# williamyang1991/VToonify

Hardware: NVIDIA H100
Metric: frames/sec at 576x1024 (higher is better)
Workload: dtype bf16x3 (fp32 operands split into bf16 hi+lo, 3 tensor-core products, fp32 accumulate)

## Files before the change

vtoonify_b200/csrc/conv_tc.cu:

```cuda
#include "tc_common.cuh"
#include <cuda_bf16.h>
#include <mutex>

using namespace vt_tc;

int vt_validate_conv_desc(const vt_conv_desc* d, const char* who);
extern int g_upfirdn_tiled;
extern int g_smalln_is;
extern int g_fir4;
extern int g_instnorm_chunks;
extern int g_rs_kernel;
int vt_conv_rs_takes(const vt_conv_desc* d);
int vt_conv_rs_run(const vt_conv_desc* d, void* stream);

namespace {

constexpr int TILE_W = 8, TILE_H = 16, TILE_M = 128;
constexpr int KCH = 32;
constexpr int MAX_SMEM = 227 * 1024;
constexpr int MAX_BLOCK_N = 128;
constexpr int MAX_ACC_COLS = 128;
constexpr int STATS_WARPS = 8;

struct TcArgs {
  CUtensorMap in_map[2][4];
  CUtensorMap w_map;
  int n_src, kchunks[2], coff[2];
  int n_steps;
  int8_t step_view[VT_MAX_TAPS], step_vx[VT_MAX_TAPS], step_vy[VT_MAX_TAPS];
  int16_t step_w[VT_MAX_TAPS];
  int step_aoff[VT_MAX_TAPS];
  int n_phase;
  int tgroup;
  int halo, halo_x0, halo_y0, halo_w;
  int n_hv, hv_view[4], hv_x0[4], hv_y0[4], hv_off[4], hv_bytes[4], a_rows;
  uint16_t step_sbo[VT_MAX_TAPS];
  int a_stages, b_stages, a_stage_bytes, b_stage_bytes, a_tx_bytes, b_tx_bytes;
  int block_n, n_tiles, tiles_x, tiles_y, B, total_tiles;
  int Ho, Wo, Cout, wB, out_cpitch;
  const float* bias;
  const float* noise;
  const float* noise_w;
  const float* res;
  float* out;
  int64_t out_sb, out_sy, out_sx, phase_off[4];
  int64_t pix_sb, pix_sy, pix_sx, phase_pix[4];
  int act, round_tf32;
  float slope, gain, alpha, beta;
  const float* rgb_w; const float* rgb_bias; const float* rgb_skip; const float* rgb_skip_kernel; float* rgb_out;
  const float* slope_vec;
  const float* src_scale[2];
  const float* src_affine[2];
  int src_cn[2];
  int64_t sc_sb, sc_sy, sc_sx;
  int in_w, in_h;
  int mma_n;
  int m_major;
  float* stats_ws;
  float acc_scale;
};

constexpr int TC_THREADS = 384;
constexpr int XFORM_WARPS = 3;
constexpr int CONSUMERS = 2;
constexpr int RELEASE_ARRIVALS = CONSUMERS * 4;

enum TcOp : int {
  OP_TF32 = 0,
  OP_BF16 = 1,
  OP_F16 = 2,
  OP_BF16_NSTACK = 3,
};

template <int NW, bool F16>
__device__ __forceinline__ void wgmma_split(float* acc, uint64_t a, uint64_t b, uint32_t accumulate) {
  if constexpr (NW == 32) {
    if constexpr (F16) wgmma_f16_n32(acc, a, b, accumulate); else wgmma_bf16_n32(acc, a, b, accumulate);
  } else if constexpr (NW == 64) {
    if constexpr (F16) wgmma_f16_n64(acc, a, b, accumulate); else wgmma_bf16_n64(acc, a, b, accumulate);
  } else {
    if constexpr (F16) wgmma_f16_n128(acc, a, b, accumulate); else wgmma_bf16_n128(acc, a, b, accumulate);
  }
}

template <int NW, int OP>
__device__ __forceinline__ void mma_step(float* acc, uint64_t adesc, uint64_t bdesc, uint32_t first) {
  if constexpr (OP == OP_TF32) {
    if constexpr (NW == 32) {
      wgmma_tf32_n32(acc, adesc, bdesc, first ^ 1u); wgmma_tf32_n32(acc, adesc + 2, bdesc + 2, 1);
      wgmma_tf32_n32(acc, adesc + 4, bdesc + 4, 1); wgmma_tf32_n32(acc, adesc + 6, bdesc + 6, 1);
    } else if constexpr (NW == 64) {
      wgmma_tf32_n64(acc, adesc, bdesc, first ^ 1u); wgmma_tf32_n64(acc, adesc + 2, bdesc + 2, 1);
      wgmma_tf32_n64(acc, adesc + 4, bdesc + 4, 1); wgmma_tf32_n64(acc, adesc + 6, bdesc + 6, 1);
    } else {
      wgmma_tf32_n128(acc, adesc, bdesc, first ^ 1u); wgmma_tf32_n128(acc, adesc + 2, bdesc + 2, 1);
      wgmma_tf32_n128(acc, adesc + 4, bdesc + 4, 1); wgmma_tf32_n128(acc, adesc + 6, bdesc + 6, 1);
    }
  } else {
    constexpr bool nstack = OP == OP_BF16_NSTACK;
    constexpr int ao[6] = {0, 2, 4, 6, 0, 2};
    constexpr int bo[6] = {0, 2, 0, 2, 4, 6};
#pragma unroll
    for (int i = 0; i < (nstack ? 4 : 6); ++i)
      wgmma_split<NW, OP == OP_F16>(acc, adesc + (uint64_t)ao[i], bdesc + (uint64_t)(nstack ? ao[i] : bo[i]), i == 0 ? (first ^ 1u) : 1u);
  }
}

template <int NW, int MT, int OP>
__global__ void __launch_bounds__(TC_THREADS, 1)
conv_tc_kernel(const __grid_constant__ TcArgs p) {
  static_assert(MT * NW <= MAX_ACC_COLS && (MT == 1 || MT == 2 || MT == 4), "accumulators of one work item exceed the register plan");
  static_assert(OP != OP_BF16_NSTACK || NW == 64, "the N-stacked form is the Cout == 32 layer at MMA N = 64");
  constexpr bool SPLIT = OP != OP_TF32;
  extern __shared__ uint8_t smem_raw[];
  const uint32_t smem_base = (smem_u32(smem_raw) + 1023u) & ~1023u;
  const uint32_t a_base = smem_base;
  const uint32_t b_base = a_base + (uint32_t)p.a_stages * p.a_stage_bytes;
  const uint32_t bar_base = b_base + (uint32_t)p.b_stages * p.b_stage_bytes;
  auto a_full = [&](int i) { return bar_base + 8u * i; };
  auto a_empty = [&](int i) { return bar_base + 64u + 8u * i; };
  auto b_full = [&](int i) { return bar_base + 128u + 8u * i; };
  auto b_empty = [&](int i) { return bar_base + 192u + 8u * i; };
  auto a_ready = [&](int i) { return bar_base + 256u + 8u * i; };

  const int warp = threadIdx.x >> 5, lane = threadIdx.x & 31;
  const int wg = threadIdx.x >> 7;

  if (warp == 0 && lane == 0) {
    for (int s = 0; s < p.n_src; ++s)
      for (int v = 0; v < 4; ++v) tma_prefetch_desc(&p.in_map[s][v]);
    tma_prefetch_desc(&p.w_map);
  }
  if (warp == 1 && lane == 0) {
    for (int i = 0; i < p.a_stages; ++i) { mbar_init(a_full(i), 1); mbar_init(a_empty(i), RELEASE_ARRIVALS); mbar_init(a_ready(i), XFORM_WARPS); }
    for (int i = 0; i < p.b_stages; ++i) { mbar_init(b_full(i), 1); mbar_init(b_empty(i), RELEASE_ARRIVALS); }
    fence_barrier_init();
    fence_proxy_async_smem();
  }
  __syncthreads();

  const int m_tiles = p.B * p.tiles_y * p.tiles_x;
  const int tiles_per_img = p.tiles_y * p.tiles_x;
  constexpr int item_w = TILE_W * MT;

  if (wg == 0) {
    if (warp == 0) {
      int a_st = 0, b_st = 0;
      uint32_t a_par = 0, b_par = 0;
      for (int tile = blockIdx.x; tile < p.total_tiles; tile += gridDim.x) {
        const int n_tile = p.m_major ? tile % p.n_tiles : tile / m_tiles, m = p.m_major ? tile / p.n_tiles : tile % m_tiles;
        const int b = m / tiles_per_img, rem = m % tiles_per_img;
        const int oy0 = (rem / p.tiles_x) * TILE_H, ox0 = (rem % p.tiles_x) * item_w;
        const int n0 = n_tile * p.block_n;
        const int wb = p.wB > 1 ? b : 0;
        for (int s = 0; s < p.n_src; ++s) {
          for (int kc = 0; kc < p.kchunks[s]; ++kc) {
            const int c0 = kc * KCH;
            if (p.halo) {
              mbar_wait(a_empty(a_st), a_par ^ 1);
              if (elect_one()) {
                const uint32_t st = a_base + a_st * p.a_stage_bytes;
                mbar_arrive_expect_tx(a_full(a_st), (uint32_t)p.a_tx_bytes);
                for (int v = 0; v < p.n_hv; ++v)
                  tma_load_4d(st + p.hv_off[v], &p.in_map[s][p.hv_view[v]], a_full(a_st), c0, ox0 + p.hv_x0[v], oy0 + p.hv_y0[v], b);
              }
              __syncwarp();
              if (++a_st == p.a_stages) { a_st = 0; a_par ^= 1; }
            }
            int gj = 0;
            for (int j = 0; j < p.n_steps; ++j) {
              if (!p.halo) {
                mbar_wait(a_empty(a_st), a_par ^ 1);
                if (elect_one()) {
// ... 6 lines not shown
              }
              if (gj == 0) {
                mbar_wait(b_empty(b_st), b_par ^ 1);
                if (elect_one()) {
                  const int wc = SPLIT ? (p.coff[s] + c0) * 2 : p.coff[s] + c0;
                  mbar_arrive_expect_tx(b_full(b_st), (uint32_t)p.b_tx_bytes);
                  tma_load_4d(b_base + b_st * p.b_stage_bytes, &p.w_map, b_full(b_st), wc, OP == OP_BF16_NSTACK ? 0 : n0, p.step_w[j], wb);
                }
                __syncwarp();
                if (++b_st == p.b_stages) { b_st = 0; b_par ^= 1; }
              }
              if (++gj == p.tgroup) gj = 0;
            }
          }
        }
      }
    } else if constexpr (SPLIT) {
      const int t = (warp - 1) * 32 + lane;
      const int rows = p.a_rows;
      int a_st = 0;
      uint32_t a_par = 0;
      const int bw = p.halo ? p.halo_w : TILE_W;
      for (int tile = blockIdx.x; tile < p.total_tiles; tile += gridDim.x) {
        const int m = p.m_major ? tile / p.n_tiles : tile % m_tiles;
        const int b = m / tiles_per_img, rem = m % tiles_per_img;
        const int oy0 = (rem / p.tiles_x) * TILE_H, ox0 = (rem % p.tiles_x) * item_w;
        for (int s = 0; s < p.n_src; ++s) {
          const float* sc = p.src_scale[s];
          const float* aff = p.src_affine[s];
          for (int kc = 0; kc < p.kchunks[s]; ++kc) {
            const float4* affp = aff ? reinterpret_cast<const float4*>(aff + ((int64_t)b * p.src_cn[s] + kc * KCH) * 2) : nullptr;
            const int loads = p.halo ? 1 : p.n_steps;
            for (int l = 0; l < loads; ++l) {
              mbar_wait(a_full(a_st), a_par);
              const uint32_t stage = a_base + a_st * p.a_stage_bytes;
              const int bx0 = ox0 + (p.halo ? p.halo_x0 : p.step_vx[l]), by0 = oy0 + (p.halo ? p.halo_y0 : p.step_vy[l]);
              for (int r = t; r < rows; r += 32 * XFORM_WARPS) {
                const uint32_t row = stage + (uint32_t)r * 128u;
                const uint32_t ph = (row >> 7) & 7u;
                float f[32];
#pragma unroll
                for (int j = 0; j < 8; ++j) {
                  float4 v;
                  asm volatile("ld.shared.v4.f32 {%0, %1, %2, %3}, [%4];" : "=f"(v.x), "=f"(v.y), "=f"(v.z), "=f"(v.w) : "r"(row + ((j ^ ph) << 4)));
                  f[4 * j] = v.x; f[4 * j + 1] = v.y; f[4 * j + 2] = v.z; f[4 * j + 3] = v.w;
                }
                if (sc || aff) {
// ... 24 lines not shown
                    const __nv_bfloat162 h2 = __floats2bfloat162_rn(f[2 * i], f[2 * i + 1]);
                    hi[i] = *reinterpret_cast<const uint32_t*>(&h2);
                    const float r0 = f[2 * i] - __uint_as_float(hi[i] << 16), r1 = f[2 * i + 1] - __uint_as_float(hi[i] & 0xffff0000u);
                    const __nv_bfloat162 l2 = __floats2bfloat162_rn(r0, r1);
                    lo[i] = *reinterpret_cast<const uint32_t*>(&l2);
                  }
                }
#pragma unroll
                for (int m4 = 0; m4 < 4; ++m4) {
                  asm volatile("st.shared.v4.b32 [%0], {%1, %2, %3, %4};" ::"r"(row + ((m4 ^ ph) << 4)), "r"(hi[4 * m4]), "r"(hi[4 * m4 + 1]), "r"(hi[4 * m4 + 2]), "r"(hi[4 * m4 + 3]) : "memory");
                  asm volatile("st.shared.v4.b32 [%0], {%1, %2, %3, %4};" ::"r"(row + (((m4 + 4) ^ ph) << 4)), "r"(lo[4 * m4]), "r"(lo[4 * m4 + 1]), "r"(lo[4 * m4 + 2]), "r"(lo[4 * m4 + 3]) : "memory");
                }
              }
              fence_proxy_async_smem();
              __syncwarp();
              if (lane == 0) mbar_arrive(a_ready(a_st));
              if (++a_st == p.a_stages) { a_st = 0; a_par ^= 1; }
            }
          }
        }
      }
    }
  } else {
    const int c = wg - 1;
    const int tw_ = (threadIdx.x & 127) >> 5;
    const bool leader = lane == 0;
    const int qd = lane & 3;
    float acc[MT][NW / 2];
#pragma unroll
    for (int g = 0; g < MT; ++g)
#pragma unroll
      for (int i = 0; i < NW / 2; ++i) acc[g][i] = 0.f;
    const float nw = (p.noise && p.noise_w) ? *p.noise_w : 0.f;
    int a_st = 0, b_st = 0;
    uint32_t a_par = 0, b_par = 0;
    const uint32_t tile_bytes_n = (uint32_t)p.mma_n * 128u;
    for (int tile = blockIdx.x; tile < p.total_tiles; tile += gridDim.x) {
      const int n_tile = p.m_major ? tile % p.n_tiles : tile / m_tiles, m = p.m_major ? tile / p.n_tiles : tile % m_tiles;
      const int b = m / tiles_per_img, rem = m % tiles_per_img;
      const int oy0 = (rem / p.tiles_x) * TILE_H, ox0 = (rem % p.tiles_x) * item_w;
      const int n0 = n_tile * p.block_n;
      uint32_t first = 1;
      int rel_a = -1, rel_b = -1;
      for (int s = 0; s < p.n_src; ++s) {
        for (int kc = 0; kc < p.kchunks[s]; ++kc) {
          if (p.halo) mbar_wait(SPLIT ? a_ready(a_st) : a_full(a_st), a_par);
          int gj = 0;
          for (int j = 0; j < p.n_steps; ++j) {
            if (!p.halo) mbar_wait(SPLIT ? a_ready(a_st) : a_full(a_st), a_par);
            if (gj == 0) mbar_wait(b_full(b_st), b_par);
            uint32_t a_addr = a_base + a_st * p.a_stage_bytes;
            uint32_t sbo = 1024;
            if (p.halo) {
              a_addr += (uint32_t)p.step_aoff[j];
              sbo = (uint32_t)p.step_sbo[j];
            }
            a_addr += 8u * (uint32_t)c * sbo;
            const uint64_t bdesc = make_smem_desc_sw128(b_base + b_st * p.b_stage_bytes + (uint32_t)gj * tile_bytes_n, 1024);
            const bool last_of_group = (gj == p.tgroup - 1);
            wgmma_fence();
#pragma unroll
// ... 52 lines not shown
          float v[2][4][2];
#pragma unroll
          for (int k = 0; k < 4; ++k)
#pragma unroll
            for (int h = 0; h < 2; ++h)
#pragma unroll
              for (int e = 0; e < 2; ++e) {
                const int i = 16 * j + 4 * k + 2 * h + e;
                float x = acc[g][i];
                if constexpr (OP == OP_BF16_NSTACK) x += acc[g][(i + 16) % (NW / 2)];
                v[h][k][e] = x * p.acc_scale;
              }
#pragma unroll
          for (int k = 0; k < 4; ++k) {
            const int ch = nb + 8 * k + 2 * qd;
            float2 bq = make_float2(0.f, 0.f), sq = make_float2(p.slope, p.slope);
            if (p.bias) bq = __ldg(reinterpret_cast<const float2*>(p.bias + ch));
            if (p.slope_vec) sq = __ldg(reinterpret_cast<const float2*>(p.slope_vec + ch));
#pragma unroll
            for (int h = 0; h < 2; ++h) {
              float v0 = v[h][k][0] + bq.x + nz[h], v1 = v[h][k][1] + bq.y + nz[h];
              if (p.act == VT_ACT_LRELU) {
                v0 = vt_lrelu(v0, sq.x) * p.gain; v1 = vt_lrelu(v1, sq.y) * p.gain;
              } else if (p.act == VT_ACT_RELU_TANH) {
                v0 = tanhf(fmaxf(v0, 0.f)); v1 = tanhf(fmaxf(v1, 0.f));
              }
              const int64_t off = p.phase_off[ph] + off0[h] + ch;
              if (p.res) {
                if (in_img[h]) {
                  const float2 rv = __ldg(reinterpret_cast<const float2*>(p.res + off));
                  v0 = v0 * p.alpha + p.beta * rv.x; v1 = v1 * p.alpha + p.beta * rv.y;
                }
              } else if (p.alpha != 1.f) {
                v0 *= p.alpha; v1 *= p.alpha;
              }
              if (p.round_tf32) { v0 = vt_round_tf32(v0); v1 = vt_round_tf32(v1); }
              if (p.rgb_w) {
                const float* w0 = p.rgb_w + ((int64_t)(p.wB > 1 ? b : 0) * 3) * p.Cout + ch;
#pragma unroll
                for (int cc = 0; cc < 3; ++cc) {
                  const float2 wv = __ldg(reinterpret_cast<const float2*>(w0 + cc * p.Cout));
                  rgb[h][cc] = fmaf(v1, wv.y, fmaf(v0, wv.x, rgb[h][cc]));
                }
              }
              if (in_img[h] && p.out) *reinterpret_cast<float2*>(p.out + off) = make_float2(v0, v1);
              v[h][k][0] = in_img[h] ? v0 : 0.f; v[h][k][1] = in_img[h] ? v1 : 0.f;
            }
          }
          if (p.stats_ws) {
            const int kchunk = ((rem * MT + g) * STATS_WARPS) + c * 4 + tw_;
            float2* wsp = reinterpret_cast<float2*>(p.stats_ws) + ((int64_t)kchunk * p.B + b) * p.Cout + nb + 2 * qd;
#pragma unroll
            for (int k = 0; k < 4; ++k)
#pragma unroll
              for (int e = 0; e < 2; ++e) {
                float ssum = v[0][k][e] + v[1][k][e];
                float ssq = fmaf(v[0][k][e], v[0][k][e], v[1][k][e] * v[1][k][e]);
#pragma unroll
                for (int o = 4; o < 32; o <<= 1) {
                  ssum += __shfl_xor_sync(0xffffffffu, ssum, o);
                  ssq += __shfl_xor_sync(0xffffffffu, ssq, o);
                }
                if (lane < 4) wsp[8 * k + e] = make_float2(ssum, ssq);
              }
          }
        }
        if (p.rgb_w) {
#pragma unroll
          for (int h = 0; h < 2; ++h)
#pragma unroll
            for (int cc = 0; cc < 3; ++cc) {
              rgb[h][cc] += __shfl_xor_sync(0xffffffffu, rgb[h][cc], 1);
              rgb[h][cc] += __shfl_xor_sync(0xffffffffu, rgb[h][cc], 2);
            }
#pragma unroll
          for (int h = 0; h < 2; ++h) {
            if (qd != 0 || !in_img[h]) continue;
            torgb_store(p.rgb_bias, p.rgb_skip, p.rgb_skip_kernel, p.rgb_out, rgb[h], b, oy[h], ox[h], p.Ho, p.Wo);
          }
        }
      }
    }
  }
}

struct TcKernel {
  int nw, mt, op;
  void (*fn)(TcArgs);
};
#define VT_TC_OPS(NW, MT) {NW, MT, OP_TF32, conv_tc_kernel<NW, MT, OP_TF32>}, {NW, MT, OP_BF16, conv_tc_kernel<NW, MT, OP_BF16>}, \
                          {NW, MT, OP_F16, conv_tc_kernel<NW, MT, OP_F16>}
const TcKernel kTcKernels[] = {
    VT_TC_OPS(128, 1), VT_TC_OPS(64, 1), VT_TC_OPS(64, 2), VT_TC_OPS(32, 1), VT_TC_OPS(32, 2), VT_TC_OPS(32, 4),
    {64, 1, OP_BF16_NSTACK, conv_tc_kernel<64, 1, OP_BF16_NSTACK>}, {64, 2, OP_BF16_NSTACK, conv_tc_kernel<64, 2, OP_BF16_NSTACK>},
};
#undef VT_TC_OPS

}

typedef CUresult (*PFN_encodeTiled)(CUtensorMap*, CUtensorMapDataType, cuuint32_t, void*, const cuuint64_t*,
                                    const cuuint64_t*, const cuuint32_t*, const cuuint32_t*, CUtensorMapInterleave,
                                    CUtensorMapSwizzle, CUtensorMapL2promotion, CUtensorMapFloatOOBfill);

static PFN_encodeTiled get_encode() {
  static PFN_encodeTiled fn = nullptr;
  static std::once_flag once;
  std::call_once(once, [] {
    void* f = nullptr;
    cudaDriverEntryPointQueryResult qres;
    if (cudaGetDriverEntryPoint("cuTensorMapEncodeTiled", &f, cudaEnableDefault, &qres) == cudaSuccess &&
        qres == cudaDriverEntryPointSuccess)
      fn = (PFN_encodeTiled)f;
  });
  return fn;
}

int vt_tc_make_map4(CUtensorMap* m, const void* base, const uint64_t dims[4], const uint64_t strides_b[3], const uint32_t box[4],
// ... 7 lines not shown
  for (int i = 0; i < 4; ++i) VT_CHECK(gd[i] >= 1 && bx[i] >= 1 && bx[i] <= 256, "conv_tc: bad %s map dim %d (dim=%llu box=%u)", what, i, (unsigned long long)gd[i], bx[i]);
  for (int i = 0; i < 3; ++i) VT_CHECK(gs[i] % 16 == 0 && gs[i] > 0, "conv_tc: %s map stride %d (%llu B) not a positive multiple of 16", what, i, (unsigned long long)gs[i]);
  VT_CHECK(((uintptr_t)base & 15) == 0, "conv_tc: %s base pointer not 16-byte aligned", what);
  CUresult r = enc(m, bf16 ? CU_TENSOR_MAP_DATA_TYPE_BFLOAT16 : CU_TENSOR_MAP_DATA_TYPE_FLOAT32, 4, const_cast<void*>(base), gd, gs, bx, es,
                   CU_TENSOR_MAP_INTERLEAVE_NONE, CU_TENSOR_MAP_SWIZZLE_128B, CU_TENSOR_MAP_L2_PROMOTION_L2_256B,
                   CU_TENSOR_MAP_FLOAT_OOB_FILL_NONE);
  VT_CHECK(r == CUDA_SUCCESS, "conv_tc: cuTensorMapEncodeTiled(%s) failed with CUresult %d", what, (int)r);
  return 0;
}


namespace {
inline int make_map4(CUtensorMap* m, const void* base, const uint64_t dims[4], const uint64_t strides_b[3], const uint32_t box[4],
                     const char* what, bool bf16 = false) { return vt_tc_make_map4(m, base, dims, strides_b, box, what, bf16); }

int g_tc_mode = 1;
int g_tc_mt = 0;
int g_tc_transpose = 1;
int g_tc_tgroup = 0;
int g_tc_s2_halo = 0;
int g_tc_stage_policy = 1;
int g_tc_halo_pct = 60;
int g_tc_m_major = 1;

int check_supported(const vt_conv_desc* d, bool set_err) {
#define VT_SUP(cond, ...) do { if (!(cond)) { if (set_err) vt_set_error(__VA_ARGS__); return 0; } } while (0)
  VT_SUP(d->Cout % 32 == 0, "conv_tc: Cout must be a multiple of 32 (got %d)", d->Cout);
  VT_SUP(d->out != nullptr || d->rgb_w != nullptr, "conv_tc: out may be NULL only with the fused ToRGB tail (image-only launch)");
  for (int s = 0; s < d->n_src; ++s) {
    VT_SUP(d->src_c[s] % KCH == 0, "conv_tc: src_c[%d]=%d must be a multiple of 32", s, d->src_c[s]);
    VT_SUP(d->src_cstride[s] % 4 == 0, "conv_tc: channel stride must be a multiple of 4");
  }
  VT_SUP(d->stride == 1 || d->stride == 2, "conv_tc: stride must be 1 or 2");
  VT_SUP(d->n_phase == 1 || (d->n_phase == 4 && d->stride == 1 && g_tc_mode != 0 && !d->res), "conv_tc: phases need stride 1, halo mode, no residual");
  for (int ph = 0; ph < d->n_phase; ++ph) VT_SUP(d->phase_off[ph] % 4 == 0, "conv_tc: phase offset must be a multiple of 4 floats");
  VT_SUP(d->out_sx % 4 == 0 && d->out_sy % 4 == 0 && d->out_sb % 4 == 0, "conv_tc: output strides must be multiples of 4 floats");
  VT_SUP(((uintptr_t)d->out & 15) == 0, "conv_tc: out not 16-byte aligned");
  VT_SUP(d->w_cstride % 4 == 0, "conv_tc: weight stride must be a multiple of 4");
  VT_SUP((!d->src_scale[0] && !d->src_scale[1] && !d->src_affine[0] && !d->src_affine[1]) || (d->weight_bf16x3 && d->stride == 1),
         "conv_tc: src_scale / src_affine need the bf16x3 mode and stride 1");
  for (int s = 0; s < 2; ++s) VT_SUP(!d->src_affine[s] || (((uintptr_t)d->src_affine[s] & 15) == 0), "conv_tc: src_affine not 16-byte aligned");
  VT_SUP(!d->bf16x3_nstack || (d->weight_bf16x3 && d->Cout == 32 && d->n_phase == 1 && d->split_fmt == 0), "conv_tc: the N-stacked bf16x3 form needs Cout == 32, one phase and the bf16 split");
  VT_SUP(d->split_fmt == 0 || d->split_fmt == 1, "conv_tc: split_fmt must be 0 (bf16) or 1 (fp16)");
  VT_SUP(!d->weight_bf16x3 || d->w_cstride % KCH == 0, "conv_tc: bf16x3 weights need a channel stride that is a multiple of 32");
  VT_SUP(!d->res || (((uintptr_t)d->res & 15) == 0), "conv_tc: res not 16-byte aligned");
  VT_SUP(!d->bias || (((uintptr_t)d->bias & 15) == 0), "conv_tc: bias not 16-byte aligned");
  VT_SUP(!d->slope_vec || (((uintptr_t)d->slope_vec & 15) == 0), "conv_tc: slope_vec not 16-byte aligned");
  VT_SUP(!d->rgb_w || (d->n_phase == 1 && d->Cout <= MAX_BLOCK_N && (d->Cout & (d->Cout - 1)) == 0 && (((uintptr_t)d->rgb_w & 15) == 0) &&
                       d->out_sx == d->Cout && d->out_sy == (int64_t)d->Wo * d->Cout && (!d->rgb_skip || (d->Ho % 2 == 0 && d->Wo % 2 == 0))),
         "conv_tc: fused ToRGB needs Cout a power of two <= 128, one phase, a dense output and even Ho/Wo for the skip");
  return 1;
#undef VT_SUP
}

}

extern "C" int vt_set_option(const char* key, int value) {
  if (key && strcmp(key, "tc_mode") == 0) { int old = g_tc_mode; g_tc_mode = value; return old; }
  if (key && strcmp(key, "tc_mt") == 0) { int old = g_tc_mt; g_tc_mt = value; return old; }
  if (key && strcmp(key, "tc_tgroup") == 0) { int old = g_tc_tgroup; g_tc_tgroup = value; return old; }
  if (key && strcmp(key, "tc_s2_halo") == 0) { int old = g_tc_s2_halo; g_tc_s2_halo = value; return old; }
  if (key && strcmp(key, "tc_stage_policy") == 0) { int old = g_tc_stage_policy; g_tc_stage_policy = value; return old; }
  if (key && strcmp(key, "tc_halo_pct") == 0) { int old = g_tc_halo_pct; g_tc_halo_pct = value; return old; }
  if (key && strcmp(key, "tc_m_major") == 0) { int old = g_tc_m_major; g_tc_m_major = value; return old; }
  if (key && strcmp(key, "tc_transpose") == 0) { int old = g_tc_transpose; g_tc_transpose = value; return old; }
  if (key && strcmp(key, "rs_kernel") == 0) { int old = g_rs_kernel; g_rs_kernel = value; return old; }
  if (key && strcmp(key, "instnorm_chunks") == 0) { int old = g_instnorm_chunks; g_instnorm_chunks = value; return old; }
  if (key && strcmp(key, "fir4") == 0) { int old = g_fir4; g_fir4 = value; return old; }
  if (key && strcmp(key, "smalln_is") == 0) { int old = g_smalln_is; g_smalln_is = value; return old; }
  if (key && strcmp(key, "upfirdn_tiled") == 0) { int old = g_upfirdn_tiled; g_upfirdn_tiled = value; return old; }
  return -1;
}

extern "C" int vt_conv2d_tc_supported(const vt_conv_desc* d) {
  if (!d || d->struct_size != (int)sizeof(vt_conv_desc)) return 0;
  return check_supported(d, false);
}

static int conv_tc_run(const vt_conv_desc* d, void* stream, int* chunks_out) {
  if (vt_validate_conv_desc(d, "conv2d_tc")) return 1;
  if (!check_supported(d, true)) return 1;

  static thread_local TcArgs a;
  memset(&a, 0, sizeof(a));

  bool T = false;
  if (g_tc_transpose && d->stride == 1 && !d->rgb_w) {
    const int64_t t0 = vt_cdiv(d->Wo, TILE_W) * vt_cdiv(d->Ho, TILE_H), t1 = vt_cdiv(d->Ho, TILE_W) * vt_cdiv(d->Wo, TILE_H);
    T = (g_tc_transpose == 2) || (t1 < t0);
  }
  const int gH = T ? d->W : d->H, gW = T ? d->H : d->W, gHo = T ? d->Wo : d->Ho, gWo = T ? d->Ho : d->Wo;
  const int64_t g_out_sy = T ? d->out_sx : d->out_sy, g_out_sx = T ? d->out_sy : d->out_sx;

  a.n_phase = d->n_phase;
  a.Ho = gHo; a.Wo = gWo; a.Cout = d->Cout; a.wB = d->wB; a.out_cpitch = d->out_cpitch;
  a.bias = d->bias; a.noise = d->noise; a.noise_w = d->noise_w; a.res = d->res;
  a.out_sb = d->out_sb; a.out_sy = g_out_sy; a.out_sx = g_out_sx;
  for (int ph = 0; ph < 4; ++ph) a.phase_off[ph] = d->phase_off[ph < d->n_phase ? ph : 0];
  if (d->noise) {
    VT_CHECK(d->out_sb % d->out_cpitch == 0 && d->out_sy % d->out_cpitch == 0 && d->out_sx % d->out_cpitch == 0,
             "conv_tc: output strides must be multiples of out_cpitch when noise is used");
    a.pix_sb = d->out_sb / d->out_cpitch; a.pix_sy = g_out_sy / d->out_cpitch; a.pix_sx = g_out_sx / d->out_cpitch;
// ... 19 lines not shown

  a.n_src = d->n_src;
  int coff = 0;
  for (int s = 0; s < d->n_src; ++s) { a.kchunks[s] = d->src_c[s] / KCH; a.coff[s] = coff; coff += d->src_c[s]; }
  a.n_steps = d->taps;
  int dxmin = 1 << 30, dxmax = -(1 << 30), dymin = 1 << 30, dymax = -(1 << 30);
  for (int t = 0; t < d->taps; ++t) {
    const int tdx = T ? d->tap_dy[t] : d->tap_dx[t], tdy = T ? d->tap_dx[t] : d->tap_dy[t];
    int view = 0, vx = tdx, vy = tdy;
    if (d->stride == 2) {
      const int px = tdx & 1, py = tdy & 1;
      view = py * 2 + px;
      vx = (tdx - px) / 2;
      vy = (tdy - py) / 2;
    }
    VT_CHECK(vx >= -100 && vx <= 100 && vy >= -100 && vy <= 100, "conv_tc: tap offset out of range");
    a.step_view[t] = (int8_t)view; a.step_vx[t] = (int8_t)vx; a.step_vy[t] = (int8_t)vy;
    a.step_w[t] = (int16_t)d->tap_w[t];
    dxmin = vx < dxmin ? vx : dxmin; dxmax = vx > dxmax ? vx : dxmax;
    dymin = vy < dymin ? vy : dymin; dymax = vy > dymax ? vy : dymax;
  }

  const int n_eff = d->n_phase * d->Cout;
  int bn = MAX_BLOCK_N;
  while (bn > 32 && (n_eff % bn) != 0) bn /= 2;
  VT_CHECK(n_eff % bn == 0, "conv_tc: no N tile for N=%d", n_eff);
  const int bnm = nstack ? 2 * bn : bn;
  const bool can_halo = (g_tc_mode != 0) && (d->taps > 1 || (bn <= 64 && d->stride == 1)) && (d->stride == 1 || g_tc_mode != 3);
  int mt = 1;
  if (can_halo && g_tc_mt != 1) {
    int want = (g_tc_mt > 0) ? g_tc_mt : (bn >= 128 ? 1 : (bn >= 64 ? 2 : 4));
    while (want > 1 && (want * bnm > MAX_ACC_COLS || gWo <= TILE_W * (want / 2))) want /= 2;
    mt = want;
  }
  const int fixed = 1024  + 1024 ;
  int smem_bytes = 0;
  int tgroup = 1;
  if (g_tc_tgroup != 1) {
    for (int tg = d->taps; tg >= 2; --tg) {
      if (d->taps % tg != 0 || tg * bnm * 128 > (g_tc_tgroup > 1 ? g_tc_tgroup : 36) * 1024) continue;
      bool ok = true;
      for (int t = 0; t < d->taps && ok; ++t)
        if (t % tg != 0 && d->tap_w[t] != d->tap_w[t - 1] + 1) ok = false;
      if (ok) { tgroup = tg; break; }
    }
  }
  a.tgroup = tgroup;
  int vx0[4], vx1[4], vy0[4], vy1[4];
  bool vused[4] = {false, false, false, false};
// ... 22 lines not shown
    const bool pays = (d->stride == 2 && g_tc_s2_halo) ? (tx_bytes * 10 <= tap_bytes * 6) : ((int64_t)tx_bytes * 100 <= tap_bytes * g_tc_halo_pct);
    a.halo = can_halo && fits && halo_bytes <= 96 * 1024 && (mt > 1 || pays) &&
             2 * halo_bytes + 2 * bnm * 128 * tgroup + fixed <= MAX_SMEM;
    if (!a.halo && mt > 1) continue;
    a.halo_x0 = a.hv_x0[0]; a.halo_y0 = a.hv_y0[0]; a.halo_w = hv_w[a.hv_view[0]];
    a.a_tx_bytes = a.halo ? tx_bytes : TILE_M * 128;
    a.a_rows = a.halo ? (a.hv_off[a.n_hv - 1] + a.hv_bytes[a.n_hv - 1]) / 128 : TILE_M;
    a.a_stage_bytes = a.halo ? halo_bytes : TILE_M * 128;
    a.b_stage_bytes = bnm * 128 * tgroup;
    a.a_stages = a.halo ? 3 : 4;
    a.b_stages = tgroup > 1 ? 4 : 6;
    const int b_floor = (g_tc_stage_policy == 1 && a.halo && a.a_stage_bytes >= 40 * 1024 && tgroup == 1) ? 5 : 3;
    while (a.a_stages * a.a_stage_bytes + a.b_stages * a.b_stage_bytes + fixed > MAX_SMEM) {
      if (a.b_stages > b_floor) --a.b_stages;
      else if (a.a_stages > 2) --a.a_stages;
      else if (a.b_stages > 2) --a.b_stages;
      else break;
    }
    if (b_floor > 3)
      while (a.b_stages < 8 && a.a_stages * a.a_stage_bytes + (a.b_stages + 1) * a.b_stage_bytes + fixed <= MAX_SMEM) ++a.b_stages;
    smem_bytes = a.a_stages * a.a_stage_bytes + a.b_stages * a.b_stage_bytes + fixed;
    if (smem_bytes <= MAX_SMEM || mt == 1) break;
  }
  a.b_tx_bytes = bnm * 128 * tgroup;
  VT_CHECK(smem_bytes <= MAX_SMEM && a.a_stages >= 2 && a.b_stages >= 2 && a.a_stages <= 8 && a.b_stages <= 8,
           "conv_tc: shared memory plan does not fit (%d B, mt=%d, bn=%d)", smem_bytes, mt, bn);
  for (int t = 0; t < d->taps; ++t) {
    const int v = a.step_view[t];
    int i = 0;
    while (i < a.n_hv - 1 && a.hv_view[i] != v) ++i;
    a.step_aoff[t] = a.hv_off[i] + ((a.step_vy[t] - vy0[v]) * hv_w[v] + (a.step_vx[t] - vx0[v])) * 128;
    a.step_sbo[t] = (uint16_t)(hv_w[v] * 128);
  }
  a.block_n = bn;
  a.mma_n = bnm;
  a.n_tiles = n_eff / bn;
  VT_CHECK(!d->rgb_w || a.n_tiles == 1, "conv_tc: fused ToRGB needs one N tile (Cout = %d)", d->Cout);
  a.tiles_x = (int)vt_cdiv(gWo, TILE_W * mt);
  a.tiles_y = (int)vt_cdiv(gHo, TILE_H);
  const int64_t total = (int64_t)a.n_tiles * a.B * a.tiles_x * a.tiles_y;
  VT_CHECK(total < (1LL << 31), "conv_tc: too many tiles");
  a.total_tiles = (int)total;
  a.m_major = g_tc_m_major ? 1 : 0;
  {
    const int64_t chunks = (int64_t)a.tiles_x * a.tiles_y * mt * STATS_WARPS;
    if (chunks_out) {
      VT_CHECK(d->n_phase == 1 && !d->rgb_w && chunks < (1 << 24), "conv_tc: output statistics need one phase and no fused ToRGB");
      *chunks_out = (int)chunks;
      return 0;
    }
    if (d->stats_ws) {
      VT_CHECK(d->n_phase == 1 && !d->rgb_w, "conv_tc: output statistics need one phase and no fused ToRGB");
      VT_CHECK(d->stats_ws_floats >= chunks * d->B * d->Cout * 2, "conv_tc: stats_ws too small (%lld floats, need %lld)",
               (long long)d->stats_ws_floats, (long long)(chunks * d->B * d->Cout * 2));
      VT_CHECK(((uintptr_t)d->stats_ws & 7) == 0, "conv_tc: stats_ws not 8-byte aligned");
      a.stats_ws = d->stats_ws;
    }
  }

  for (int s = 0; s < d->n_src; ++s) {
    const uint64_t cs = (uint64_t)d->src_cstride[s];
    if (d->stride == 1) {
      const uint64_t real_sx = cs * 4, real_sy = (uint64_t)d->W * cs * 4;
      const uint64_t dims[4] = {cs, (uint64_t)gW, (uint64_t)gH, (uint64_t)d->B};
      const uint64_t str[3] = {T ? real_sy : real_sx, T ? real_sx : real_sy, (uint64_t)d->H * d->W * cs * 4};
// ... 24 lines not shown
      VT_CHECK(((uintptr_t)d->weight_bf16x3 & 15) == 0, "conv_tc: weight_bf16x3 not 16-byte aligned");
      const uint64_t rows = (uint64_t)n_eff * (nstack ? 2 : 1);
      const uint64_t dims2[4] = {2 * wc, rows, (uint64_t)d->w_taps, (uint64_t)d->wB};
      const uint64_t str2[3] = {wc * 4, rows * wc * 4, (uint64_t)d->w_taps * rows * wc * 4};
      const uint32_t box[4] = {2 * KCH, (uint32_t)bnm, (uint32_t)a.tgroup, 1};
      if (make_map4(&a.w_map, d->weight_bf16x3, dims2, str2, box, "weight(bf16x3)", true)) return 1;
    } else {
      const uint32_t box[4] = {KCH, (uint32_t)bn, (uint32_t)a.tgroup, 1};
      if (make_map4(&a.w_map, d->weight, dims, str, box, "weight")) return 1;
    }
  }
  static std::once_flag attr_once;
  static cudaError_t attr_err = cudaSuccess;
  std::call_once(attr_once, [] {
    for (const TcKernel& k : kTcKernels)
      if (attr_err == cudaSuccess) attr_err = cudaFuncSetAttribute(k.fn, cudaFuncAttributeMaxDynamicSharedMemorySize, MAX_SMEM);
  });
  VT_CHECK(attr_err == cudaSuccess, "conv_tc: cudaFuncSetAttribute failed: %s", cudaGetErrorString(attr_err));
  const TcKernel* kern = nullptr;
  for (const TcKernel& k : kTcKernels)
    if (k.nw == bnm && k.mt == mt && k.op == op) kern = &k;
  if (!kern) return vt_set_error("conv_tc: no kernel for MMA N = %d, %d M tiles, operand mode %d", bnm, mt, op);
  int grid = vt_num_sms();
  if (grid > a.total_tiles) grid = a.total_tiles;
  kern->fn<<<grid, TC_THREADS, smem_bytes, (cudaStream_t)stream>>>(a);
  VT_LAUNCH_CHECK();
  return 0;
}

extern "C" int vt_conv2d_tc_tf32(const vt_conv_desc* d, void* stream) { return conv_tc_run(d, stream, nullptr); }

static bool rs_shape(const vt_conv_desc* d) {
  if (d->n_src != 1 || d->stride != 1 || d->taps != 9 || d->n_phase != 1 || d->res || d->slope_vec || !d->weight_bf16x3) return false;
  if (d->src_scale[0] || d->src_affine[0] || d->alpha != 1.f) return false;
  if ((d->Cout != 32 && d->Cout != 64) || (d->src_c[0] != 32 && d->src_c[0] != 64)) return false;
  return d->act == VT_ACT_NONE || d->act == VT_ACT_LRELU;
}

extern "C" int vt_conv2d_rs_supported(const vt_conv_desc* d) {
  if (!d || d->struct_size != (int)sizeof(vt_conv_desc)) return 0;
  return rs_shape(d) && check_supported(d, false);
}

extern "C" int vt_conv2d_rs(const vt_conv_desc* d, float acc_scale, void* stream) {
  VT_CHECK(d && d->struct_size == (int)sizeof(vt_conv_desc) && rs_shape(d), "conv2d_rs: not a row-strip layer (3x3, stride 1, Cin/Cout in {32, 64})");
  vt_conv_desc c = *d;
  if (acc_scale > 0.f) c.acc_scale = acc_scale;
  if (g_rs_kernel && vt_conv_rs_takes(&c)) return vt_conv_rs_run(&c, stream);
  return conv_tc_run(&c, stream, nullptr);
}
// ... 8 lines not shown
```

vtoonify_b200/csrc/wgmma_sm90.cuh:

```cuda
#pragma once
#include <stdint.h>

namespace vt_tc {

__device__ __forceinline__ void wgmma_tf32_n32(float* d, uint64_t a, uint64_t b, uint32_t accumulate) {
  asm volatile(
      "{\n\t.reg .pred p;\n\tsetp.ne.b32 p, %18, 0;\n\t"
      "wgmma.mma_async.sync.aligned.m64n32k8.f32.tf32.tf32 "
      "{%0, %1, %2, %3, %4, %5, %6, %7, %8, %9, %10, %11, %12, %13, %14, %15}, %16, %17, p, 1, 1;\n\t}"
      : "+f"(d[0]), "+f"(d[1]), "+f"(d[2]), "+f"(d[3]), "+f"(d[4]), "+f"(d[5]), "+f"(d[6]), "+f"(d[7]), "+f"(d[8]), "+f"(d[9]), "+f"(d[10]), "+f"(d[11]), "+f"(d[12]), "+f"(d[13]), "+f"(d[14]), "+f"(d[15])
      : "l"(a), "l"(b), "r"(accumulate));
}
__device__ __forceinline__ void wgmma_bf16_n32(float* d, uint64_t a, uint64_t b, uint32_t accumulate) {
  asm volatile(
      "{\n\t.reg .pred p;\n\tsetp.ne.b32 p, %18, 0;\n\t"
      "wgmma.mma_async.sync.aligned.m64n32k16.f32.bf16.bf16 "
      "{%0, %1, %2, %3, %4, %5, %6, %7, %8, %9, %10, %11, %12, %13, %14, %15}, %16, %17, p, 1, 1, 0, 0;\n\t}"
      : "+f"(d[0]), "+f"(d[1]), "+f"(d[2]), "+f"(d[3]), "+f"(d[4]), "+f"(d[5]), "+f"(d[6]), "+f"(d[7]), "+f"(d[8]), "+f"(d[9]), "+f"(d[10]), "+f"(d[11]), "+f"(d[12]), "+f"(d[13]), "+f"(d[14]), "+f"(d[15])
      : "l"(a), "l"(b), "r"(accumulate));
}
__device__ __forceinline__ void wgmma_f16_n32(float* d, uint64_t a, uint64_t b, uint32_t accumulate) {
  asm volatile(
      "{\n\t.reg .pred p;\n\tsetp.ne.b32 p, %18, 0;\n\t"
      "wgmma.mma_async.sync.aligned.m64n32k16.f32.f16.f16 "
// ... 29 lines not shown
  asm volatile(
      "{\n\t.reg .pred p;\n\tsetp.ne.b32 p, %66, 0;\n\t"
      "wgmma.mma_async.sync.aligned.m64n128k8.f32.tf32.tf32 "
      "{%0, %1, %2, %3, %4, %5, %6, %7, %8, %9, %10, %11, %12, %13, %14, %15, %16, %17, %18, %19, %20, %21, %22, %23, %24, %25, %26, %27, %28, %29, %30, %31, %32, %33, %34, %35, %36, %37, %38, %39, %40, %41, %42, %43, %44, %45, %46, %47, %48, %49, %50, %51, %52, %53, %54, %55, %56, %57, %58, %59, %60, %61, %62, %63}, %64, %65, p, 1, 1;\n\t}"
      : "+f"(d[0]), "+f"(d[1]), "+f"(d[2]), "+f"(d[3]), "+f"(d[4]), "+f"(d[5]), "+f"(d[6]), "+f"(d[7]), "+f"(d[8]), "+f"(d[9]), "+f"(d[10]), "+f"(d[11]), "+f"(d[12]), "+f"(d[13]), "+f"(d[14]), "+f"(d[15]), "+f"(d[16]), "+f"(d[17]), "+f"(d[18]), "+f"(d[19]), "+f"(d[20]), "+f"(d[21]), "+f"(d[22]), "+f"(d[23]), "+f"(d[24]), "+f"(d[25]), "+f"(d[26]), "+f"(d[27]), "+f"(d[28]), "+f"(d[29]), "+f"(d[30]), "+f"(d[31]), "+f"(d[32]), "+f"(d[33]), "+f"(d[34]), "+f"(d[35]), "+f"(d[36]), "+f"(d[37]), "+f"(d[38]), "+f"(d[39]), "+f"(d[40]), "+f"(d[41]), "+f"(d[42]), "+f"(d[43]), "+f"(d[44]), "+f"(d[45]), "+f"(d[46]), "+f"(d[47]), "+f"(d[48]), "+f"(d[49]), "+f"(d[50]), "+f"(d[51]), "+f"(d[52]), "+f"(d[53]), "+f"(d[54]), "+f"(d[55]), "+f"(d[56]), "+f"(d[57]), "+f"(d[58]), "+f"(d[59]), "+f"(d[60]), "+f"(d[61]), "+f"(d[62]), "+f"(d[63])
      : "l"(a), "l"(b), "r"(accumulate));
}
__device__ __forceinline__ void wgmma_bf16_n128(float* d, uint64_t a, uint64_t b, uint32_t accumulate) {
  asm volatile(
      "{\n\t.reg .pred p;\n\tsetp.ne.b32 p, %66, 0;\n\t"
      "wgmma.mma_async.sync.aligned.m64n128k16.f32.bf16.bf16 "
      "{%0, %1, %2, %3, %4, %5, %6, %7, %8, %9, %10, %11, %12, %13, %14, %15, %16, %17, %18, %19, %20, %21, %22, %23, %24, %25, %26, %27, %28, %29, %30, %31, %32, %33, %34, %35, %36, %37, %38, %39, %40, %41, %42, %43, %44, %45, %46, %47, %48, %49, %50, %51, %52, %53, %54, %55, %56, %57, %58, %59, %60, %61, %62, %63}, %64, %65, p, 1, 1, 0, 0;\n\t}"
      : "+f"(d[0]), "+f"(d[1]), "+f"(d[2]), "+f"(d[3]), "+f"(d[4]), "+f"(d[5]), "+f"(d[6]), "+f"(d[7]), "+f"(d[8]), "+f"(d[9]), "+f"(d[10]), "+f"(d[11]), "+f"(d[12]), "+f"(d[13]), "+f"(d[14]), "+f"(d[15]), "+f"(d[16]), "+f"(d[17]), "+f"(d[18]), "+f"(d[19]), "+f"(d[20]), "+f"(d[21]), "+f"(d[22]), "+f"(d[23]), "+f"(d[24]), "+f"(d[25]), "+f"(d[26]), "+f"(d[27]), "+f"(d[28]), "+f"(d[29]), "+f"(d[30]), "+f"(d[31]), "+f"(d[32]), "+f"(d[33]), "+f"(d[34]), "+f"(d[35]), "+f"(d[36]), "+f"(d[37]), "+f"(d[38]), "+f"(d[39]), "+f"(d[40]), "+f"(d[41]), "+f"(d[42]), "+f"(d[43]), "+f"(d[44]), "+f"(d[45]), "+f"(d[46]), "+f"(d[47]), "+f"(d[48]), "+f"(d[49]), "+f"(d[50]), "+f"(d[51]), "+f"(d[52]), "+f"(d[53]), "+f"(d[54]), "+f"(d[55]), "+f"(d[56]), "+f"(d[57]), "+f"(d[58]), "+f"(d[59]), "+f"(d[60]), "+f"(d[61]), "+f"(d[62]), "+f"(d[63])
      : "l"(a), "l"(b), "r"(accumulate));
}
__device__ __forceinline__ void wgmma_f16_n128(float* d, uint64_t a, uint64_t b, uint32_t accumulate) {
  asm volatile(
      "{\n\t.reg .pred p;\n\tsetp.ne.b32 p, %66, 0;\n\t"
      "wgmma.mma_async.sync.aligned.m64n128k16.f32.f16.f16 "
      "{%0, %1, %2, %3, %4, %5, %6, %7, %8, %9, %10, %11, %12, %13, %14, %15, %16, %17, %18, %19, %20, %21, %22, %23, %24, %25, %26, %27, %28, %29, %30, %31, %32, %33, %34, %35, %36, %37, %38, %39, %40, %41, %42, %43, %44, %45, %46, %47, %48, %49, %50, %51, %52, %53, %54, %55, %56, %57, %58, %59, %60, %61, %62, %63}, %64, %65, p, 1, 1, 0, 0;\n\t}"
      : "+f"(d[0]), "+f"(d[1]), "+f"(d[2]), "+f"(d[3]), "+f"(d[4]), "+f"(d[5]), "+f"(d[6]), "+f"(d[7]), "+f"(d[8]), "+f"(d[9]), "+f"(d[10]), "+f"(d[11]), "+f"(d[12]), "+f"(d[13]), "+f"(d[14]), "+f"(d[15]), "+f"(d[16]), "+f"(d[17]), "+f"(d[18]), "+f"(d[19]), "+f"(d[20]), "+f"(d[21]), "+f"(d[22]), "+f"(d[23]), "+f"(d[24]), "+f"(d[25]), "+f"(d[26]), "+f"(d[27]), "+f"(d[28]), "+f"(d[29]), "+f"(d[30]), "+f"(d[31]), "+f"(d[32]), "+f"(d[33]), "+f"(d[34]), "+f"(d[35]), "+f"(d[36]), "+f"(d[37]), "+f"(d[38]), "+f"(d[39]), "+f"(d[40]), "+f"(d[41]), "+f"(d[42]), "+f"(d[43]), "+f"(d[44]), "+f"(d[45]), "+f"(d[46]), "+f"(d[47]), "+f"(d[48]), "+f"(d[49]), "+f"(d[50]), "+f"(d[51]), "+f"(d[52]), "+f"(d[53]), "+f"(d[54]), "+f"(d[55]), "+f"(d[56]), "+f"(d[57]), "+f"(d[58]), "+f"(d[59]), "+f"(d[60]), "+f"(d[61]), "+f"(d[62]), "+f"(d[63])
      : "l"(a), "l"(b), "r"(accumulate));
}

__device__ __forceinline__ void wgmma_fence() { asm volatile("wgmma.fence.sync.aligned;" ::: "memory"); }
__device__ __forceinline__ void wgmma_commit() { asm volatile("wgmma.commit_group.sync.aligned;" ::: "memory"); }
template <int N>
__device__ __forceinline__ void wgmma_wait() { asm volatile("wgmma.wait_group.sync.aligned %0;" ::"n"(N) : "memory"); }
template <int R>
__device__ __forceinline__ void wgmma_pin(float* d) {
#pragma unroll
  for (int i = 0; i < R; ++i) asm volatile("" : "+f"(d[i])::"memory");
}

}
```

Measured before the change: 34.68.

## Add 256-wide bf16 MMA tile with register rebalancing and tail-wave split launch

```diff
diff --git a/vtoonify_b200/csrc/conv_tc.cu b/vtoonify_b200/csrc/conv_tc.cu
--- a/vtoonify_b200/csrc/conv_tc.cu
+++ b/vtoonify_b200/csrc/conv_tc.cu
@@ -20,6 +20,9 @@
 constexpr int MAX_SMEM = 227 * 1024;
 constexpr int MAX_BLOCK_N = 128;
 constexpr int MAX_ACC_COLS = 128;
+constexpr int WIDE_N = 256;
+constexpr int WIDE_REGS_XFORM = 88;
+constexpr int WIDE_REGS_CONSUMER = 208;
 constexpr int STATS_WARPS = 8;
 
 struct TcArgs {
@@ -37,6 +40,7 @@
   uint16_t step_sbo[VT_MAX_TAPS];
   int a_stages, b_stages, a_stage_bytes, b_stage_bytes, a_tx_bytes, b_tx_bytes;
   int block_n, n_tiles, tiles_x, tiles_y, B, total_tiles;
+  int m_first;
   int Ho, Wo, Cout, wB, out_cpitch;
   const float* bias;
   const float* noise;
@@ -78,8 +82,11 @@
     if constexpr (F16) wgmma_f16_n32(acc, a, b, accumulate); else wgmma_bf16_n32(acc, a, b, accumulate);
   } else if constexpr (NW == 64) {
     if constexpr (F16) wgmma_f16_n64(acc, a, b, accumulate); else wgmma_bf16_n64(acc, a, b, accumulate);
+  } else if constexpr (NW == 128) {
+    if constexpr (F16) wgmma_f16_n128(acc, a, b, accumulate); else wgmma_bf16_n128(acc, a, b, accumulate);
   } else {
-    if constexpr (F16) wgmma_f16_n128(acc, a, b, accumulate); else wgmma_bf16_n128(acc, a, b, accumulate);
+    static_assert(NW == WIDE_N && !F16, "the 256-wide MMA exists for the bf16 split only");
+    wgmma_bf16_n256(acc, a, b, accumulate);
   }
 }
 
@@ -109,7 +116,11 @@
 template <int NW, int MT, int OP>
 __global__ void __launch_bounds__(TC_THREADS, 1)
 conv_tc_kernel(const __grid_constant__ TcArgs p) {
-  static_assert(MT * NW <= MAX_ACC_COLS && (MT == 1 || MT == 2 || MT == 4), "accumulators of one work item exceed the register plan");
+  constexpr bool WIDE = NW == WIDE_N;
+  static_assert((MT * NW <= MAX_ACC_COLS || (WIDE && MT == 1 && OP == OP_BF16)) && (MT == 1 || MT == 2 || MT == 4),
+                "accumulators of one work item exceed the register plan");
+  static_assert(128 * WIDE_REGS_XFORM + 256 * WIDE_REGS_CONSUMER <= TC_THREADS * ((65536 / TC_THREADS) & ~7),
+                "setmaxnreg plan exceeds the launch allocation");
   static_assert(OP != OP_BF16_NSTACK || NW == 64, "the N-stacked form is the Cout == 32 layer at MMA N = 64");
   constexpr bool SPLIT = OP != OP_TF32;
   extern __shared__ uint8_t smem_raw[];
@@ -139,16 +150,17 @@
   }
   __syncthreads();
 
-  const int m_tiles = p.B * p.tiles_y * p.tiles_x;
+  const int m_tiles = p.total_tiles / p.n_tiles;
   const int tiles_per_img = p.tiles_y * p.tiles_x;
   constexpr int item_w = TILE_W * MT;
 
   if (wg == 0) {
+    if constexpr (WIDE) asm volatile("setmaxnreg.dec.sync.aligned.u32 %0;" ::"n"(WIDE_REGS_XFORM));
     if (warp == 0) {
       int a_st = 0, b_st = 0;
       uint32_t a_par = 0, b_par = 0;
       for (int tile = blockIdx.x; tile < p.total_tiles; tile += gridDim.x) {
-        const int n_tile = p.m_major ? tile % p.n_tiles : tile / m_tiles, m = p.m_major ? tile / p.n_tiles : tile % m_tiles;
+        const int n_tile = p.m_major ? tile % p.n_tiles : tile / m_tiles, m = p.m_first + (p.m_major ? tile / p.n_tiles : tile % m_tiles);
         const int b = m / tiles_per_img, rem = m % tiles_per_img;
         const int oy0 = (rem / p.tiles_x) * TILE_H, ox0 = (rem % p.tiles_x) * item_w;
         const int n0 = n_tile * p.block_n;
@@ -201,7 +213,7 @@
       uint32_t a_par = 0;
       const int bw = p.halo ? p.halo_w : TILE_W;
       for (int tile = blockIdx.x; tile < p.total_tiles; tile += gridDim.x) {
-        const int m = p.m_major ? tile / p.n_tiles : tile % m_tiles;
+        const int m = p.m_first + (p.m_major ? tile / p.n_tiles : tile % m_tiles);
         const int b = m / tiles_per_img, rem = m % tiles_per_img;
         const int oy0 = (rem / p.tiles_x) * TILE_H, ox0 = (rem % p.tiles_x) * item_w;
         for (int s = 0; s < p.n_src; ++s) {
@@ -272,6 +284,7 @@
       }
     }
   } else {
+    if constexpr (WIDE) asm volatile("setmaxnreg.inc.sync.aligned.u32 %0;" ::"n"(WIDE_REGS_CONSUMER));
     const int c = wg - 1;
     const int tw_ = (threadIdx.x & 127) >> 5;
     const bool leader = lane == 0;
@@ -286,7 +299,7 @@
     uint32_t a_par = 0, b_par = 0;
     const uint32_t tile_bytes_n = (uint32_t)p.mma_n * 128u;
     for (int tile = blockIdx.x; tile < p.total_tiles; tile += gridDim.x) {
-      const int n_tile = p.m_major ? tile % p.n_tiles : tile / m_tiles, m = p.m_major ? tile / p.n_tiles : tile % m_tiles;
+      const int n_tile = p.m_major ? tile % p.n_tiles : tile / m_tiles, m = p.m_first + (p.m_major ? tile / p.n_tiles : tile % m_tiles);
       const int b = m / tiles_per_img, rem = m % tiles_per_img;
       const int oy0 = (rem / p.tiles_x) * TILE_H, ox0 = (rem % p.tiles_x) * item_w;
       const int n0 = n_tile * p.block_n;
@@ -385,7 +398,7 @@
               float v0 = v[h][k][0] + bq.x + nz[h], v1 = v[h][k][1] + bq.y + nz[h];
               if (p.act == VT_ACT_LRELU) {
                 v0 = vt_lrelu(v0, sq.x) * p.gain; v1 = vt_lrelu(v1, sq.y) * p.gain;
-              } else if (p.act == VT_ACT_RELU_TANH) {
+              } else if (!WIDE && p.act == VT_ACT_RELU_TANH) {
                 v0 = tanhf(fmaxf(v0, 0.f)); v1 = tanhf(fmaxf(v1, 0.f));
               }
               const int64_t off = p.phase_off[ph] + off0[h] + ch;
@@ -398,7 +411,7 @@
                 v0 *= p.alpha; v1 *= p.alpha;
               }
               if (p.round_tf32) { v0 = vt_round_tf32(v0); v1 = vt_round_tf32(v1); }
-              if (p.rgb_w) {
+              if (!WIDE && p.rgb_w) {
                 const float* w0 = p.rgb_w + ((int64_t)(p.wB > 1 ? b : 0) * 3) * p.Cout + ch;
 #pragma unroll
                 for (int cc = 0; cc < 3; ++cc) {
@@ -428,7 +441,7 @@
               }
           }
         }
-        if (p.rgb_w) {
+        if (!WIDE && p.rgb_w) {
 #pragma unroll
           for (int h = 0; h < 2; ++h)
 #pragma unroll
@@ -456,6 +469,7 @@
 const TcKernel kTcKernels[] = {
     VT_TC_OPS(128, 1), VT_TC_OPS(64, 1), VT_TC_OPS(64, 2), VT_TC_OPS(32, 1), VT_TC_OPS(32, 2), VT_TC_OPS(32, 4),
     {64, 1, OP_BF16_NSTACK, conv_tc_kernel<64, 1, OP_BF16_NSTACK>}, {64, 2, OP_BF16_NSTACK, conv_tc_kernel<64, 2, OP_BF16_NSTACK>},
+    {WIDE_N, 1, OP_BF16, conv_tc_kernel<WIDE_N, 1, OP_BF16>},
 };
 #undef VT_TC_OPS
 
@@ -509,6 +523,7 @@
 int g_tc_stage_policy = 1;
 int g_tc_halo_pct = 60;
 int g_tc_m_major = 1;
+int g_tc_wide = 1;
 
 int check_supported(const vt_conv_desc* d, bool set_err) {
 #define VT_SUP(cond, ...) do { if (!(cond)) { if (set_err) vt_set_error(__VA_ARGS__); return 0; } } while (0)
@@ -551,6 +566,7 @@
   if (key && strcmp(key, "tc_halo_pct") == 0) { int old = g_tc_halo_pct; g_tc_halo_pct = value; return old; }
   if (key && strcmp(key, "tc_m_major") == 0) { int old = g_tc_m_major; g_tc_m_major = value; return old; }
   if (key && strcmp(key, "tc_transpose") == 0) { int old = g_tc_transpose; g_tc_transpose = value; return old; }
+  if (key && strcmp(key, "tc_wide") == 0) { int old = g_tc_wide; g_tc_wide = value; return old; }
   if (key && strcmp(key, "rs_kernel") == 0) { int old = g_rs_kernel; g_rs_kernel = value; return old; }
   if (key && strcmp(key, "instnorm_chunks") == 0) { int old = g_instnorm_chunks; g_instnorm_chunks = value; return old; }
   if (key && strcmp(key, "fir4") == 0) { int old = g_fir4; g_fir4 = value; return old; }
@@ -564,7 +580,7 @@
   return check_supported(d, false);
 }
 
-static int conv_tc_run(const vt_conv_desc* d, void* stream, int* chunks_out) {
+static int conv_tc_run(const vt_conv_desc* d, void* stream, int* chunks_out, int m_first = 0, bool allow_wide = true) {
   if (vt_validate_conv_desc(d, "conv2d_tc")) return 1;
   if (!check_supported(d, true)) return 1;
 
@@ -630,9 +646,12 @@
   }
 
   const int n_eff = d->n_phase * d->Cout;
-  int bn = MAX_BLOCK_N;
-  while (bn > 32 && (n_eff % bn) != 0) bn /= 2;
-  VT_CHECK(n_eff % bn == 0, "conv_tc: no N tile for N=%d", n_eff);
+  int bn_narrow = MAX_BLOCK_N;
+  while (bn_narrow > 32 && (n_eff % bn_narrow) != 0) bn_narrow /= 2;
+  VT_CHECK(n_eff % bn_narrow == 0, "conv_tc: no N tile for N=%d", n_eff);
+  const bool wide = allow_wide && (g_tc_wide == 2 || (g_tc_wide == 1 && d->stride == 1)) && op == OP_BF16 && n_eff % WIDE_N == 0 &&
+                    !d->rgb_w && d->act != VT_ACT_RELU_TANH;
+  const int bn = wide ? WIDE_N : bn_narrow;
   const int bnm = nstack ? 2 * bn : bn;
   const bool can_halo = (g_tc_mode != 0) && (d->taps > 1 || (bn <= 64 && d->stride == 1)) && (d->stride == 1 || g_tc_mode != 3);
   int mt = 1;
@@ -701,6 +720,7 @@
     smem_bytes = a.a_stages * a.a_stage_bytes + a.b_stages * a.b_stage_bytes + fixed;
     if (smem_bytes <= MAX_SMEM || mt == 1) break;
   }
+  if (wide && !(smem_bytes <= MAX_SMEM && a.a_stages >= 2 && a.b_stages >= 3)) return conv_tc_run(d, stream, chunks_out, m_first, false);
   a.b_tx_bytes = bnm * 128 * tgroup;
   VT_CHECK(smem_bytes <= MAX_SMEM && a.a_stages >= 2 && a.b_stages >= 2 && a.a_stages <= 8 && a.b_stages <= 8,
            "conv_tc: shared memory plan does not fit (%d B, mt=%d, bn=%d)", smem_bytes, mt, bn);
@@ -717,9 +737,12 @@
   VT_CHECK(!d->rgb_w || a.n_tiles == 1, "conv_tc: fused ToRGB needs one N tile (Cout = %d)", d->Cout);
   a.tiles_x = (int)vt_cdiv(gWo, TILE_W * mt);
   a.tiles_y = (int)vt_cdiv(gHo, TILE_H);
-  const int64_t total = (int64_t)a.n_tiles * a.B * a.tiles_x * a.tiles_y;
+  const int64_t m_total = (int64_t)a.B * a.tiles_x * a.tiles_y;
+  VT_CHECK(m_first < m_total, "conv_tc: first pixel tile %d out of range", m_first);
+  const int64_t total = (int64_t)a.n_tiles * (m_total - m_first);
   VT_CHECK(total < (1LL << 31), "conv_tc: too many tiles");
   a.total_tiles = (int)total;
+  a.m_first = m_first;
   a.m_major = g_tc_m_major ? 1 : 0;
   {
     const int64_t chunks = (int64_t)a.tiles_x * a.tiles_y * mt * STATS_WARPS;
@@ -790,10 +813,14 @@
     if (k.nw == bnm && k.mt == mt && k.op == op) kern = &k;
   if (!kern) return vt_set_error("conv_tc: no kernel for MMA N = %d, %d M tiles, operand mode %d", bnm, mt, op);
   int grid = vt_num_sms();
+  int m_split = 0;
+  if (wide && g_tc_wide == 1 && a.total_tiles >= grid && a.total_tiles % grid != 0)
+    m_split = (a.total_tiles / grid) * grid / a.n_tiles;
+  if (m_split > 0) a.total_tiles = m_split * a.n_tiles;
   if (grid > a.total_tiles) grid = a.total_tiles;
   kern->fn<<<grid, TC_THREADS, smem_bytes, (cudaStream_t)stream>>>(a);
   VT_LAUNCH_CHECK();
-  return 0;
+  return m_split > 0 ? conv_tc_run(d, stream, nullptr, m_split, false) : 0;
 }
 
 extern "C" int vt_conv2d_tc_tf32(const vt_conv_desc* d, void* stream) { return conv_tc_run(d, stream, nullptr); }
diff --git a/vtoonify_b200/csrc/wgmma_sm90.cuh b/vtoonify_b200/csrc/wgmma_sm90.cuh
--- a/vtoonify_b200/csrc/wgmma_sm90.cuh
+++ b/vtoonify_b200/csrc/wgmma_sm90.cuh
@@ -75,6 +75,14 @@
       : "+f"(d[0]), "+f"(d[1]), "+f"(d[2]), "+f"(d[3]), "+f"(d[4]), "+f"(d[5]), "+f"(d[6]), "+f"(d[7]), "+f"(d[8]), "+f"(d[9]), "+f"(d[10]), "+f"(d[11]), "+f"(d[12]), "+f"(d[13]), "+f"(d[14]), "+f"(d[15]), "+f"(d[16]), "+f"(d[17]), "+f"(d[18]), "+f"(d[19]), "+f"(d[20]), "+f"(d[21]), "+f"(d[22]), "+f"(d[23]), "+f"(d[24]), "+f"(d[25]), "+f"(d[26]), "+f"(d[27]), "+f"(d[28]), "+f"(d[29]), "+f"(d[30]), "+f"(d[31]), "+f"(d[32]), "+f"(d[33]), "+f"(d[34]), "+f"(d[35]), "+f"(d[36]), "+f"(d[37]), "+f"(d[38]), "+f"(d[39]), "+f"(d[40]), "+f"(d[41]), "+f"(d[42]), "+f"(d[43]), "+f"(d[44]), "+f"(d[45]), "+f"(d[46]), "+f"(d[47]), "+f"(d[48]), "+f"(d[49]), "+f"(d[50]), "+f"(d[51]), "+f"(d[52]), "+f"(d[53]), "+f"(d[54]), "+f"(d[55]), "+f"(d[56]), "+f"(d[57]), "+f"(d[58]), "+f"(d[59]), "+f"(d[60]), "+f"(d[61]), "+f"(d[62]), "+f"(d[63])
       : "l"(a), "l"(b), "r"(accumulate));
 }
+__device__ __forceinline__ void wgmma_bf16_n256(float* d, uint64_t a, uint64_t b, uint32_t accumulate) {
+  asm volatile(
+      "{\n\t.reg .pred p;\n\tsetp.ne.b32 p, %130, 0;\n\t"
+      "wgmma.mma_async.sync.aligned.m64n256k16.f32.bf16.bf16 "
+      "{%0, %1, %2, %3, %4, %5, %6, %7, %8, %9, %10, %11, %12, %13, %14, %15, %16, %17, %18, %19, %20, %21, %22, %23, %24, %25, %26, %27, %28, %29, %30, %31, %32, %33, %34, %35, %36, %37, %38, %39, %40, %41, %42, %43, %44, %45, %46, %47, %48, %49, %50, %51, %52, %53, %54, %55, %56, %57, %58, %59, %60, %61, %62, %63, %64, %65, %66, %67, %68, %69, %70, %71, %72, %73, %74, %75, %76, %77, %78, %79, %80, %81, %82, %83, %84, %85, %86, %87, %88, %89, %90, %91, %92, %93, %94, %95, %96, %97, %98, %99, %100, %101, %102, %103, %104, %105, %106, %107, %108, %109, %110, %111, %112, %113, %114, %115, %116, %117, %118, %119, %120, %121, %122, %123, %124, %125, %126, %127}, %128, %129, p, 1, 1, 0, 0;\n\t}"
+      : "+f"(d[0]), "+f"(d[1]), "+f"(d[2]), "+f"(d[3]), "+f"(d[4]), "+f"(d[5]), "+f"(d[6]), "+f"(d[7]), "+f"(d[8]), "+f"(d[9]), "+f"(d[10]), "+f"(d[11]), "+f"(d[12]), "+f"(d[13]), "+f"(d[14]), "+f"(d[15]), "+f"(d[16]), "+f"(d[17]), "+f"(d[18]), "+f"(d[19]), "+f"(d[20]), "+f"(d[21]), "+f"(d[22]), "+f"(d[23]), "+f"(d[24]), "+f"(d[25]), "+f"(d[26]), "+f"(d[27]), "+f"(d[28]), "+f"(d[29]), "+f"(d[30]), "+f"(d[31]), "+f"(d[32]), "+f"(d[33]), "+f"(d[34]), "+f"(d[35]), "+f"(d[36]), "+f"(d[37]), "+f"(d[38]), "+f"(d[39]), "+f"(d[40]), "+f"(d[41]), "+f"(d[42]), "+f"(d[43]), "+f"(d[44]), "+f"(d[45]), "+f"(d[46]), "+f"(d[47]), "+f"(d[48]), "+f"(d[49]), "+f"(d[50]), "+f"(d[51]), "+f"(d[52]), "+f"(d[53]), "+f"(d[54]), "+f"(d[55]), "+f"(d[56]), "+f"(d[57]), "+f"(d[58]), "+f"(d[59]), "+f"(d[60]), "+f"(d[61]), "+f"(d[62]), "+f"(d[63]), "+f"(d[64]), "+f"(d[65]), "+f"(d[66]), "+f"(d[67]), "+f"(d[68]), "+f"(d[69]), "+f"(d[70]), "+f"(d[71]), "+f"(d[72]), "+f"(d[73]), "+f"(d[74]), "+f"(d[75]), "+f"(d[76]), "+f"(d[77]), "+f"(d[78]), "+f"(d[79]), "+f"(d[80]), "+f"(d[81]), "+f"(d[82]), "+f"(d[83]), "+f"(d[84]), "+f"(d[85]), "+f"(d[86]), "+f"(d[87]), "+f"(d[88]), "+f"(d[89]), "+f"(d[90]), "+f"(d[91]), "+f"(d[92]), "+f"(d[93]), "+f"(d[94]), "+f"(d[95]), "+f"(d[96]), "+f"(d[97]), "+f"(d[98]), "+f"(d[99]), "+f"(d[100]), "+f"(d[101]), "+f"(d[102]), "+f"(d[103]), "+f"(d[104]), "+f"(d[105]), "+f"(d[106]), "+f"(d[107]), "+f"(d[108]), "+f"(d[109]), "+f"(d[110]), "+f"(d[111]), "+f"(d[112]), "+f"(d[113]), "+f"(d[114]), "+f"(d[115]), "+f"(d[116]), "+f"(d[117]), "+f"(d[118]), "+f"(d[119]), "+f"(d[120]), "+f"(d[121]), "+f"(d[122]), "+f"(d[123]), "+f"(d[124]), "+f"(d[125]), "+f"(d[126]), "+f"(d[127])
+      : "l"(a), "l"(b), "r"(accumulate));
+}
 
 __device__ __forceinline__ void wgmma_fence() { asm volatile("wgmma.fence.sync.aligned;" ::: "memory"); }
 __device__ __forceinline__ void wgmma_commit() { asm volatile("wgmma.commit_group.sync.aligned;" ::: "memory"); }
```

After: 36.98, median of 6. 1.07x the previous value.
